# feiyuhuahuo/Yolact_minimal

Measured on NVIDIA B200. Metric: img/s, higher is better.
Workload: dtype f16

## Files before the change

yolact_minimal_b200/csrc/conv_tc.cu:

```cuda
#include "layers.cuh"

#include <cuda.h>
#include <cuda_fp16.h>
#include <stdlib.h>
#include <string.h>
#include <mutex>

namespace yb {

constexpr int TC_BM = 128;
constexpr int TC_BK = 64;
constexpr int TC_THREADS = 320;
constexpr int TC_OUT_BUFS = 2;
constexpr uint32_t TC_WARP_TILE = 32 * 32 * 2;
constexpr uint32_t TC_A_STAGE = TC_BM * TC_BK * 2;
constexpr uint32_t TC_SLAB_ROWS = TC_BM + 2;
constexpr uint32_t TC_A_SLAB = 136 * TC_BK * 2;
constexpr uint32_t TC_S16_ROWS = TC_BM + 3;
constexpr uint32_t TC_S16_SLOT = 5120;

struct TcParams {
  long long M;
  int m_tiles, n_tiles;
  int kb_per_tap;
  int ntaps;
  int tap_shift[kMaxTaps];
  int BN;
  int tmem_cols;
  int stages;
  int Cout, Cout_pad, relu, out_mode;
  int is_f16;
  int tma_epi;
  int nres;
  int b_resident;
  int slab, stages_a;
  int alt_tiles;
  int res_kb;
  int stem16;
  int gemm;
  int gemm_ntile_tap;
  int gemm_shift[16];
  int accumulate;
  int gemm_splits;
  int gemm_kb_split;
  Geom g;
  const float* bias;
  const void* residual;
  void* out;
};

struct TcPlan {
  CUtensorMap tmA, tmB, tmOut, tmRes;
  int BN, stages, tmem_cols, tma_epi, nres, b_resident, res_kb, pair, slab, stages_a, alt_tiles, stem16;
  int sms;
  int gemm;
  size_t smem_bytes;
};

__device__ __forceinline__ uint32_t smem_u32(const void* p) { return (uint32_t)__cvta_generic_to_shared(p); }

__device__ __forceinline__ void mbar_init(uint64_t* bar, uint32_t count) {
  asm volatile("mbarrier.init.shared::cta.b64 [%0], %1;" ::"r"(smem_u32(bar)), "r"(count));
}
__device__ __forceinline__ void mbar_expect_tx(uint64_t* bar, uint32_t bytes) {
  asm volatile("mbarrier.arrive.expect_tx.shared::cta.b64 _, [%0], %1;" ::"r"(smem_u32(bar)), "r"(bytes) : "memory");
}
__device__ __forceinline__ void mbar_arrive(uint64_t* bar) {
  asm volatile("mbarrier.arrive.shared::cta.b64 _, [%0];" ::"r"(smem_u32(bar)) : "memory");
}
__device__ __forceinline__ void mbar_wait(uint64_t* bar, uint32_t parity) {
  asm volatile(
      "{\n\t.reg .pred p;\n\t"
      "WAIT_LOOP:\n\t"
      "mbarrier.try_wait.parity.shared::cta.b64 p, [%0], %1;\n\t"
      "@p bra WAIT_DONE;\n\t"
      "bra WAIT_LOOP;\n\t"
      "WAIT_DONE:\n\t}" ::"r"(smem_u32(bar)), "r"(parity)
// ... 115 lines not shown
__device__ __forceinline__ void tmem_ld16(uint32_t taddr, uint32_t* r) {
  asm volatile(
      "tcgen05.ld.sync.aligned.32x32b.x16.b32 {%0,%1,%2,%3,%4,%5,%6,%7,%8,%9,%10,%11,%12,%13,%14,%15}, [%16];"
      : "=r"(r[0]), "=r"(r[1]), "=r"(r[2]), "=r"(r[3]), "=r"(r[4]), "=r"(r[5]), "=r"(r[6]), "=r"(r[7]), "=r"(r[8]),
        "=r"(r[9]), "=r"(r[10]), "=r"(r[11]), "=r"(r[12]), "=r"(r[13]), "=r"(r[14]), "=r"(r[15])
      : "r"(taddr)
      : "memory");
}
__device__ __forceinline__ void tmem_ld_wait() { asm volatile("tcgen05.wait::ld.sync.aligned;" ::: "memory"); }

template <bool F16> __device__ __forceinline__ uint32_t pack2(float a, float b) {
  if (F16) {
    __half2 v = __floats2half2_rn(fminf(fmaxf(a, -65504.f), 65504.f), fminf(fmaxf(b, -65504.f), 65504.f));
    return *reinterpret_cast<uint32_t*>(&v);
  } else {
    __nv_bfloat162 v = __floats2bfloat162_rn(a, b);
    return *reinterpret_cast<uint32_t*>(&v);
  }
}
template <bool F16, bool RELU> __device__ __forceinline__ uint32_t pack2_sat(float a, float b) {
  uint32_t r;
  if (F16) {
    if (RELU) asm("cvt.rn.relu.satfinite.f16x2.f32 %0, %1, %2;" : "=r"(r) : "f"(b), "f"(a));
    else asm("cvt.rn.satfinite.f16x2.f32 %0, %1, %2;" : "=r"(r) : "f"(b), "f"(a));
  } else {
    if (RELU) asm("cvt.rn.relu.bf16x2.f32 %0, %1, %2;" : "=r"(r) : "f"(b), "f"(a));
    else asm("cvt.rn.bf16x2.f32 %0, %1, %2;" : "=r"(r) : "f"(b), "f"(a));
  }
  return r;
}
template <bool F16> __device__ __forceinline__ float2 unpack2(uint32_t u) {
  if (F16) return __half22float2(*reinterpret_cast<const __half2*>(&u));
  return __bfloat1622float2(*reinterpret_cast<const __nv_bfloat162*>(&u));
}

template <int NCOL, bool F16>
__device__ __forceinline__ void epilogue_chunk(const TcParams& p, const uint32_t* acc, long long m, int col, bool valid, bool halo,
                                               int img, int y, int x) {
  if (!valid) return;
  if (p.out_mode == 2) {
    float* o = (float*)p.out + m * p.Cout_pad + col;
#pragma unroll
    for (int i = 0; i < NCOL; i += 4) {
      const float4 r = make_float4(__uint_as_float(acc[i]), __uint_as_float(acc[i + 1]), __uint_as_float(acc[i + 2]), __uint_as_float(acc[i + 3]));
      if (p.accumulate) atomicAdd(reinterpret_cast<float4*>(o + i), r);
      else *reinterpret_cast<float4*>(o + i) = r;
    }
    return;
  }
  float v[NCOL];
#pragma unroll
  for (int i = 0; i < NCOL; i += 4) {
    const float4 b = __ldg(reinterpret_cast<const float4*>(p.bias + col + i));
    v[i] = __uint_as_float(acc[i]) + b.x; v[i + 1] = __uint_as_float(acc[i + 1]) + b.y;
    v[i + 2] = __uint_as_float(acc[i + 2]) + b.z; v[i + 3] = __uint_as_float(acc[i + 3]) + b.w;
  }
  if (p.out_mode == 0) {
    uint16_t* o = (uint16_t*)p.out + m * p.Cout + col;
    if (halo) {
#pragma unroll
      for (int i = 0; i < NCOL; i += 8) *reinterpret_cast<uint4*>(o + i) = make_uint4(0, 0, 0, 0);
      return;
    }
    if (p.residual) {
      const uint16_t* r = (const uint16_t*)p.residual + m * p.Cout + col;
#pragma unroll
// ... 340 lines not shown
      mbar_expect_tx(&gres_full[buf], TC_WARP_TILE);
      tma_load_2d(gRes + buf * TC_WARP_TILE, &tmRes, pf_nt * p.BN + (2 * pf_j + grp) * 32, pf_mt * TC_BM + quad * 32, &gres_full[buf]);
      ++pf_seq;
      if (++pf_j == my_chunks) { pf_j = 0; ++pf_it; pf_ok = tile_at<PAIR>(p, pf_it, pf_mt, pf_nt); }
    };
    if (elected) {
      for (int q = 0; q < nres && pf_ok; ++q) issue_res_load();
    }
    int m_tile, n_tile;
    for (int it = 0; tile_at<PAIR>(p, it, m_tile, n_tile); ++it) {
      if (p.alt_tiles && (it & 1) != grp) {
        acc ^= 1; if (acc == 0) acc_phase ^= 1;
        continue;
      }
      const long long m = (long long)m_tile * TC_BM + row_in_tile;
      const bool valid = m < p.M;
      int img = 0, y = 0, x = 0;
      bool halo = false;
      if (valid && p.out_mode != 2) {
        const int plane = p.g.plane();
        img = (int)(m / plane);
        const int pos = (int)(m - (long long)img * plane);
        y = pos / p.g.Wp(); x = pos - y * p.g.Wp();
        halo = y == 0 || y == p.g.H + 1 || x == 0 || x == p.g.W + 1;
      }
      mbar_wait(&tmem_full[acc], acc_phase);
      tc_fence_after();
      const uint32_t t_base = tmem_base + ((uint32_t)(quad * 32) << 16) + (uint32_t)(acc * p.BN);
      const int n0 = n_tile * p.BN;
      if (p.tma_epi) {
        const uint32_t sw = (uint32_t)((lane >> 1) & 3);
        const bool zero_row = halo || !valid;
        const int row0 = m_tile * TC_BM + quad * 32;
        uint32_t r[32];
        if (my_chunks > 0) tmem_ld32(t_base + cfirst * 32, r);
        for (int j = 0; j < my_chunks; ++j, ++seq) {
          const int c = cstep * j + cfirst;
          const int col = n0 + c * 32;
          const int obuf = seq & (TC_OUT_BUFS - 1);
          float v[32];
#pragma unroll
          for (int i = 0; i < 32; i += 4) {
            const float4 b = __ldg(reinterpret_cast<const float4*>(p.bias + col + i));
            v[i] = b.x; v[i + 1] = b.y; v[i + 2] = b.z; v[i + 3] = b.w;
          }
          tmem_ld_wait();
#pragma unroll
          for (int i = 0; i < 32; ++i) v[i] += __uint_as_float(r[i]);
          if (j + 1 < my_chunks) tmem_ld32(t_base + (c + cstep) * 32, r);
          if (has_res) {
            const int rbuf = seq & (nres - 1);
            mbar_wait(&gres_full[rbuf], (uint32_t)((seq >> nres_shift) & 1));
            const uint8_t* rrow = gRes + rbuf * TC_WARP_TILE + lane * 64;
#pragma unroll
            for (int jj = 0; jj < 4; ++jj) {
              const uint4 rv = *reinterpret_cast<const uint4*>(rrow + (((uint32_t)jj ^ sw) << 4));
              const uint32_t rw[4] = {rv.x, rv.y, rv.z, rv.w};
#pragma unroll
              for (int q = 0; q < 4; ++q) {
                const float2 f = unpack2<F16>(rw[q]);
                v[jj * 8 + 2 * q] += f.x; v[jj * 8 + 2 * q + 1] += f.y;
              }
            }
          }
          uint32_t pk[16];
          if (p.relu == 1) {
#pragma unroll
            for (int i = 0; i < 16; ++i) pk[i] = pack2_sat<F16, true>(v[2 * i], v[2 * i + 1]);
          } else {
            if (p.relu == 2) {
#pragma unroll
              for (int i = 0; i < 32; ++i) v[i] = apply_act(v[i], 2);
            }
#pragma unroll
            for (int i = 0; i < 16; ++i) pk[i] = pack2_sat<F16, false>(v[2 * i], v[2 * i + 1]);
          }
          if (zero_row) {
#pragma unroll
            for (int i = 0; i < 16; ++i) pk[i] = 0u;
          }
          if (elected) bulk_wait_read<1>();
          __syncwarp();
          uint8_t* orow = gOut + obuf * TC_WARP_TILE + lane * 64;
#pragma unroll
          for (int jj = 0; jj < 4; ++jj)
            *reinterpret_cast<uint4*>(orow + (((uint32_t)jj ^ sw) << 4)) = make_uint4(pk[jj * 4], pk[jj * 4 + 1], pk[jj * 4 + 2], pk[jj * 4 + 3]);
          fence_async_smem();
          __syncwarp();
          if (elected) {
            tma_store_2d(&tmOut, gOut + obuf * TC_WARP_TILE, col, row0);
            bulk_commit();
            if (pf_ok) issue_res_load();
          }
        }
      } else {
        for (int c0 = cfirst * 32; c0 < p.BN; c0 += 32 * cstep) {
          uint32_t r[32];
          if (c0 + 32 <= p.BN) {
            tmem_ld32(t_base + c0, r);
            tmem_ld_wait();
            epilogue_chunk<32, F16>(p, r, m, n0 + c0, valid, halo, img, y, x);
          } else {
            tmem_ld16(t_base + c0, r);
            tmem_ld_wait();
            epilogue_chunk<16, F16>(p, r, m, n0 + c0, valid, halo, img, y, x);
          }
        }
      }
      tc_fence_before();
      __syncwarp();
      if (lane == 0) {
        if (PAIR) mbar_arrive_cluster(map_to_rank(smem_u32(&tmem_empty[acc]), 0)); else mbar_arrive(&tmem_empty[acc]);
      }
      acc ^= 1; if (acc == 0) acc_phase ^= 1;
    }
    if (p.tma_epi && elected) bulk_wait<0>();
  }

  tc_fence_before();
  if (PAIR) cluster_sync_all(); else __syncthreads();
  if (warp == 1) {
    tc_fence_after();
// ... 569 lines not shown
  p.ntaps = 1; p.tap_shift[0] = 0;
  for (int i = 0; i < g.ntaps; ++i) p.gemm_shift[i] = g.shift[i];
  p.BN = pl->BN; p.tmem_cols = pl->tmem_cols; p.stages = pl->stages;
  p.Cout = p.Cout_pad = g.ntaps * g.Nper; p.relu = 0; p.out_mode = 2; p.accumulate = g.accumulate;
  p.is_f16 = g.act_dt == DT_F16; p.alt_tiles = pl->alt_tiles;
  p.g.H = 1 << 20; p.g.W = 1 << 20;
  p.bias = nullptr; p.residual = nullptr; p.out = g.out;
  const int total = p.m_tiles * p.n_tiles * p.gemm_splits;
  const int grid = total < pl->sms ? total : pl->sms;
  cudaLaunchConfig_t cfg = {};
  cfg.gridDim = dim3((unsigned)grid); cfg.blockDim = dim3(TC_THREADS); cfg.dynamicSmemBytes = pl->smem_bytes; cfg.stream = s;
  cfg.attrs = nullptr; cfg.numAttrs = 0;
  const cudaError_t le = p.is_f16 ? cudaLaunchKernelEx(&cfg, k_conv_tc<true, false>, pl->tmA, pl->tmB, pl->tmOut, pl->tmRes, p)
                                  : cudaLaunchKernelEx(&cfg, k_conv_tc<false, false>, pl->tmA, pl->tmB, pl->tmOut, pl->tmRes, p);
  YB_CHECK_CUDA(le);
  YB_CHECK_LAUNCH();
  return YB_OK;
}

int launch_conv_tc(const TcPlan* pl, const ConvArgs& a, cudaStream_t s) {
  TcParams p;
  p.M = (long long)a.B * a.g.plane();
  const int unit_rows = pl->pair ? 2 * TC_BM : TC_BM;
  p.m_tiles = (int)((p.M + unit_rows - 1) / unit_rows);
  p.n_tiles = a.Cout_pad / pl->BN;
  p.kb_per_tap = a.Cin_pad / TC_BK;
  p.ntaps = a.ntaps;
  for (int i = 0; i < kMaxTaps; ++i) p.tap_shift[i] = a.tap_shift[i];
  p.BN = pl->BN; p.tmem_cols = pl->tmem_cols; p.stages = pl->stages;
  p.Cout = a.Cout; p.Cout_pad = a.Cout_pad; p.relu = a.relu; p.out_mode = a.out_mode;
  p.g = a.g; p.bias = a.bias; p.residual = a.residual; p.out = a.out; p.is_f16 = a.act_dt == DT_F16; p.tma_epi = pl->tma_epi; p.nres = pl->nres; p.b_resident = pl->b_resident; p.res_kb = pl->res_kb; p.slab = pl->slab; p.stages_a = pl->stages_a; p.alt_tiles = pl->alt_tiles; p.stem16 = pl->stem16;
  p.gemm = 0; p.gemm_ntile_tap = 1; p.accumulate = 0; p.gemm_splits = 1; p.gemm_kb_split = 0;
  for (int i = 0; i < 16; ++i) p.gemm_shift[i] = 0;
  const int sms = pl->sms;
  const int total = p.m_tiles * p.n_tiles;
  const int max_units = pl->pair ? sms / 2 : sms;
  int units = total < max_units ? total : max_units;
  if (pl->b_resident) {
    units = max_units / p.n_tiles * p.n_tiles;
    if (units > total) units = total;
    if (units < p.n_tiles) units = p.n_tiles;
  }
  const int grid = pl->pair ? 2 * units : units;
  static const bool pdl = getenv("YOLACT_B200_NO_PDL") == nullptr;
  cudaLaunchConfig_t cfg = {};
  cfg.gridDim = dim3((unsigned)grid); cfg.blockDim = dim3(TC_THREADS); cfg.dynamicSmemBytes = pl->smem_bytes; cfg.stream = s;
  cudaLaunchAttribute attr[2];
  int na = 0;
  if (pdl) {
    attr[na].id = cudaLaunchAttributeProgrammaticStreamSerialization;
    attr[na].val.programmaticStreamSerializationAllowed = 1;
    ++na;
  }
  if (pl->pair) {
    attr[na].id = cudaLaunchAttributeClusterDimension;
    attr[na].val.clusterDim.x = 2; attr[na].val.clusterDim.y = 1; attr[na].val.clusterDim.z = 1;
    ++na;
  }
  cfg.attrs = attr; cfg.numAttrs = na;
  cudaError_t le;
  if (pl->pair) le = p.is_f16 ? cudaLaunchKernelEx(&cfg, k_conv_tc<true, true>, pl->tmA, pl->tmB, pl->tmOut, pl->tmRes, p)
                              : cudaLaunchKernelEx(&cfg, k_conv_tc<false, true>, pl->tmA, pl->tmB, pl->tmOut, pl->tmRes, p);
  else le = p.is_f16 ? cudaLaunchKernelEx(&cfg, k_conv_tc<true, false>, pl->tmA, pl->tmB, pl->tmOut, pl->tmRes, p)
                     : cudaLaunchKernelEx(&cfg, k_conv_tc<false, false>, pl->tmA, pl->tmB, pl->tmOut, pl->tmRes, p);
  YB_CHECK_CUDA(le);
  YB_CHECK_LAUNCH();
// ... 96 lines not shown
```

yolact_minimal_b200/csrc/kernels_simt.cu:

```cuda
#include "layers.cuh"
#include <mutex>
#include "vecio.cuh"
#include <math.h>
#include <algorithm>

namespace yb {

__device__ __forceinline__ bool is_halo(long long m, const Geom& g, int& n, int& y, int& x) {
  const int plane = g.plane();
  n = (int)(m / plane);
  const int pos = (int)(m - (long long)n * plane);
  y = pos / g.Wp();
  x = pos - y * g.Wp();
  return y == 0 || y == g.H + 1 || x == 0 || x == g.W + 1;
}

constexpr int SBM = 64, SBN = 64, SBK = 16;

template <typename T>
__global__ void __launch_bounds__(256) k_conv_simt(ConvArgs a, long long M) {
  __shared__ float As[SBK][SBM + 4];
  __shared__ float Bs[SBK][SBN + 4];
  const int tid = threadIdx.x;
  const long long m0 = (long long)blockIdx.x * SBM;
// ... 38 lines not shown
      }
    }
  }
  const T* res = (const T*)a.residual;
#pragma unroll
  for (int i = 0; i < 4; ++i) {
    const long long m = m0 + ty * 4 + i;
    if (m >= M) continue;
    int n, y, x;
    const bool halo = is_halo(m, a.g, n, y, x);
#pragma unroll
    for (int j = 0; j < 4; ++j) {
      const int c = n0 + tx * 4 + j;
      if (c >= a.Cout_pad) continue;
      float v = acc[i][j] + a.bias[c];
      if (a.out_mode == 0) {
        if (c >= a.Cout) continue;
        if (res) v += Act<T>::ld(res + m * a.Cout + c);
        v = apply_act(v, a.relu);
        Act<T>::st((T*)a.out + m * a.Cout + c, halo ? 0.f : v);
      } else if (!halo) {
        v = apply_act(v, a.relu);
        const long long r = ((long long)n * a.g.H + (y - 1)) * a.g.W + (x - 1);
        ((float*)a.out)[r * a.Cout_pad + c] = v;
      }
    }
  }
}

int launch_conv_simt(const ConvArgs& a, cudaStream_t s) {
  const long long M = (long long)a.B * a.g.plane();
  dim3 grid((unsigned)((M + SBM - 1) / SBM), (unsigned)ceil_div(a.Cout_pad, SBN));
  YB_REQUIRE(a.Cin % 4 == 0 && a.Cin_pad % SBK == 0, YB_ERR_UNSUPPORTED, "conv_simt: Cin=%d / Cin_pad=%d", a.Cin, a.Cin_pad);
  YB_DISPATCH_DT(a.act_dt, (k_conv_simt<T><<<grid, 256, 0, s>>>(a, M)));
  YB_CHECK_LAUNCH();
  return YB_OK;
}

constexpr int ST = 16;
constexpr int SP = ST * 2 + 5;

template <typename T>
__global__ void __launch_bounds__(256) k_stem(const float* __restrict__ img, const float* __restrict__ w,
                                              const float* __restrict__ bias, T* __restrict__ out, int S, int H1) {
  extern __shared__ float sm[];
  float* s_w = sm;
  float* s_in = sm + 147 * 64;
  const int tid = threadIdx.x, b = blockIdx.z;
  const int oy0 = blockIdx.y * ST, ox0 = blockIdx.x * ST;
  for (int i = tid; i < 147 * 64; i += 256) s_w[i] = w[i];
  const int iy0 = oy0 * 2 - 3, ix0 = ox0 * 2 - 3;
  for (int i = tid; i < 3 * SP * SP; i += 256) {
    const int c = i / (SP * SP), r = (i / SP) % SP, q = i % SP;
    const int iy = iy0 + r, ix = ix0 + q;
    float v = 0.f;
    if (iy >= 0 && iy < S && ix >= 0 && ix < S) v = img[(((size_t)b * 3 + c) * S + iy) * S + ix];
    s_in[(c * SP + r) * (SP + 1) + q] = v;
  }
  __syncthreads();
  const int py = tid / ST, px = tid % ST;
  const int oy = oy0 + py, ox = ox0 + px;
  float acc[64];
#pragma unroll
  for (int c = 0; c < 64; ++c) acc[c] = 0.f;
  for (int r = 0; r < 7; ++r)
    for (int q = 0; q < 7; ++q)
// ... 458 lines not shown
```

yolact_minimal_b200/csrc/layers.cuh:

```cuda
#pragma once
#include "common.cuh"
#include <cuda_fp16.h>

namespace yb {

enum DType { DT_F32 = 0, DT_BF16 = 1, DT_F16 = 2 };
static inline size_t dtype_size(int dt) { return dt == DT_F32 ? 4 : 2; }

struct Geom {
  int H, W;
  __host__ __device__ int Hp() const { return H + 2; }
  __host__ __device__ int Wp() const { return W + 2; }
  __host__ __device__ int plane() const { return Hp() * Wp(); }
};

constexpr int kMaxTaps = 9;

struct ConvArgs {
  const void* in;
  const void* weight;
  const float* bias;
  const void* residual;
  void* out;
  int act_dt;
  int B;
  Geom g;
  int Cin, Cout, Cout_pad;
  int Cin_pad;
  int ntaps;
  int tap_shift[kMaxTaps];
  int relu;
  int out_mode;
  long long in_rows;
  int in_row_stride;
  long long w_ld;
};

#define YB_DISPATCH_DT(dt, ...)                                   \
  do {                                                            \
    if ((dt) == DT_F32) { using T = float; __VA_ARGS__; }         \
    else if ((dt) == DT_BF16) { using T = __nv_bfloat16; __VA_ARGS__; } \
    else { using T = __half; __VA_ARGS__; }                       \
  } while (0)

int launch_conv_simt(const ConvArgs& a, cudaStream_t s);

struct TcPlan;
int tc_plan_create(const ConvArgs& a_maxbatch, int max_batch, TcPlan** out);
void tc_plan_destroy(TcPlan* p);
int launch_conv_tc(const TcPlan* p, const ConvArgs& a, cudaStream_t s);
bool tc_supported(const ConvArgs& a);

struct GemmArgs {
  const void* a; const void* b; float* out;
  int act_dt, M, Nper, K, lda, ldb, ntaps, accumulate;
  int splits;
  long long Kb;
  int shift[16];
};
int tc_plan_create_gemm(const GemmArgs& g, TcPlan** out);
int launch_gemm_tc(const TcPlan* p, const GemmArgs& g, cudaStream_t s);

struct BneckArgs {
  const void* t2; const void* x; const void* w3; const void* w1;
  const void* xd; int Cd;
  const float* b3; const float* b1;
  void* xo; void* t1;
  int act_dt, B, Cmid, Cexp;
// ... 32 lines not shown
```

yolact_minimal_b200/csrc/net.cu:

```cuda
#include "layers.cuh"

#include <math.h>
#include <stdlib.h>
#include <string.h>
#include <algorithm>
#include <map>
#include <memory>
#include <string>
#include <vector>

using namespace yb;

namespace {

struct Param {
  std::string name;
  int64_t count;
  std::vector<float> data;
  bool set = false;
};

struct ActBuf {
  int C = 0, H = 0;
  int planes = 1;
// ... 1 lines not shown
  size_t bytes = 0;
  int first = 0, last = 0;
  int slot = -1;
  bool dense_f32 = false;
  int pad_rows = 0;
};

enum OpKind { OP_STEM, OP_POOL, OP_SPLIT, OP_CONV, OP_UPADD, OP_UP2X, OP_HEADFIN, OP_PATCH_EMBED, OP_LN, OP_ATTN, OP_MERGE_LN, OP_BNECK };
enum ExtOut { EXT_NONE = 0, EXT_PROTO = 1 };

struct ConvW {
  std::string wname, bname, bnname;
  std::vector<std::string> cat;
  int Cin = 0, Cin_pad = 0, Cout = 0, Cout_pad = 0, k = 1;
  void* d_w = nullptr;
  float* d_b = nullptr;
};

struct Op {
  OpKind kind;
  int in = -1, out = -1, res = -1;
  int conv = -1;
  int stride = 1, relu = 0, out_mode = 0, ext = EXT_NONE;
  int level = 0;
  int aux = -1;
  std::string p0, p1, p2;
  int heads = 0, shift = 0;
  TcPlan* tc = nullptr;
  int conv2 = -1, out2 = -1;
  BnPlan* bn = nullptr;
  int convd = -1, in2 = -1;
  void* d_wcat = nullptr;
  float* d_bcat = nullptr;
};

}

struct yb_net {
  yb_net_config cfg{};
  std::vector<Param> params;
  std::map<std::string, int> pidx;
  std::vector<ActBuf> acts;
  std::vector<ConvW> convs;
  std::vector<Op> ops;
  std::vector<Op> ops_base;
  std::map<std::string, int> taps;
  std::vector<void*> slots;
  std::vector<size_t> slot_bytes;
  bool finalized = false;
  int max_batch = 0, precision = 0, act_dt = DT_F32;
  int H1 = 0, H2 = 0;
  int level_size[5]{}, level_off[5]{};
  int A = 0, P = 0;
  std::vector<float> anchors;
  float* d_anchors = nullptr;
  float* d_stem_w = nullptr;
  float* d_stem_b = nullptr;
  std::map<std::string, float*> d_vec;
  float* d_pe_w = nullptr;
  void* d_stem_w16 = nullptr;
  int stem_wide = 0;
  float* d_stem_b16 = nullptr;
  ConvArgs stem_args{};
  float *d_img = nullptr, *d_cls = nullptr, *d_box = nullptr, *d_coef = nullptr, *d_proto = nullptr;
  void* d_ws = nullptr; size_t ws_bytes = 0;
  int32_t *d_cnt = nullptr, *d_ocls = nullptr, *d_oanc = nullptr; float *d_osc = nullptr, *d_obox = nullptr, *d_ocoef = nullptr;
// ... 245 lines not shown
      const bool ok = ca.k == 1 && cb.k == 1 && a.stride == 1 && b.stride == 1 && a.res >= 0 && b.res < 0 && a.relu == 1 && b.relu == 1 &&
                      a.out_mode == 0 && b.out_mode == 0 && a.ext == EXT_NONE && b.ext == EXT_NONE && b.in == a.out && ca.cat.empty() &&
                      cb.cat.empty() && ca.Cout == cb.Cin && cb.Cout == ca.Cin && ca.Cin == ca.Cin_pad && cb.Cin == cb.Cin_pad &&
                      ca.Cout == ca.Cout_pad && cb.Cout == cb.Cout_pad && bneck_supported(net->act_dt, ca.Cin, ca.Cout);
      if (ok) {
        Op f = a;
        f.kind = OP_BNECK; f.conv2 = b.conv; f.out2 = b.out;
        merged.push_back(f);
        ++i;
        continue;
      }
    }
    merged.push_back(a);
  }
  std::vector<Op> folded;
  for (size_t i = 0; i < merged.size(); ++i) {
    Op f = merged[i];
    if (f.kind == OP_BNECK && !folded.empty() && !getenv("YOLACT_B200_NO_FUSE_DOWN")) {
      const Op& d = folded.back();
      if (d.kind == OP_CONV && d.out == f.res && d.stride == 1 && d.relu == 0 && d.res < 0 && d.out_mode == 0 && d.ext == EXT_NONE) {
        const ConvW& cd = net->convs[d.conv];
        const ConvW& c3 = net->convs[f.conv];
        if (cd.k == 1 && cd.cat.empty() && cd.Cin == cd.Cin_pad && cd.Cout == c3.Cout && (c3.Cin + cd.Cin) / 64 <= 2 && net->acts[d.in].H == net->acts[f.in].H) {
          f.convd = d.conv; f.in2 = d.in; f.res = -1;
          folded.pop_back();
        }
      }
    }
    folded.push_back(f);
  }
  net->ops.swap(folded);
}

void bneck_args(const yb_net* net, const Op& o, int B, BneckArgs* a) {
  const ConvW& c3 = net->convs[o.conv];
  const ConvW& c1 = net->convs[o.conv2];
  memset(a, 0, sizeof(*a));
  a->t2 = net->slots[net->acts[o.in].slot];
  if (o.convd >= 0) { a->xd = net->slots[net->acts[o.in2].slot]; a->Cd = net->convs[o.convd].Cin; }
  else a->x = net->slots[net->acts[o.res].slot];
  a->xo = net->slots[net->acts[o.out].slot]; a->t1 = net->slots[net->acts[o.out2].slot];
  a->w3 = o.convd >= 0 ? o.d_wcat : c3.d_w; a->b3 = o.convd >= 0 ? o.d_bcat : c3.d_b; a->w1 = c1.d_w; a->b1 = c1.d_b;
  a->act_dt = net->act_dt; a->B = B; a->Cmid = c3.Cin; a->Cexp = c3.Cout;
  a->g.H = net->acts[o.in].H; a->g.W = a->g.H;
}

void plan_memory(yb_net* net) {
  auto& acts = net->acts;
  for (auto& a : acts) { a.first = 1 << 30; a.last = -1; }
  for (int i = 0; i < (int)net->ops.size(); ++i) {
    const Op& o = net->ops[i];
    for (int t : {o.in, o.out, o.res, o.aux, o.out2, o.in2}) {
      if (t < 0) continue;
      acts[t].first = acts[t].first < i ? acts[t].first : i;
      acts[t].last = acts[t].last > i ? acts[t].last : i;
    }
  }
  for (auto& kv : net->taps) acts[kv.second].last = 1 << 30;
  const size_t esz = dtype_size(net->act_dt);
  for (auto& a : acts) {
    a.dt = a.dense_f32 ? DT_F32 : net->act_dt;
    const size_t rows = a.dense_f32 ? (size_t)net->max_batch * a.H * a.H : (size_t)net->max_batch * (a.H + 2) * (a.H + 2) * a.planes;
    a.bytes = align_up((rows + a.pad_rows) * a.C * (a.dense_f32 ? 4 : esz), 1024);
  }
  std::vector<int> slot_free_at;
  net->slot_bytes.clear();
// ... 59 lines not shown
      for (int co = 0; co < cout; ++co) bias[row + co] = bb[co];
      row += cout;
    }
  }
  if (net->act_dt == DT_F32) {
    YB_PROPAGATE(upload(w.data(), w.size() * 4, &c.d_w));
  } else if (net->act_dt == DT_BF16) {
    std::vector<__nv_bfloat16> wb(w.size());
    for (size_t i = 0; i < w.size(); ++i) wb[i] = __float2bfloat16_rn(w[i]);
    YB_PROPAGATE(upload(wb.data(), wb.size() * 2, &c.d_w));
  } else {
    std::vector<__half> wb(w.size());
    for (size_t i = 0; i < w.size(); ++i) wb[i] = __float2half_rn(w[i]);
    YB_PROPAGATE(upload(wb.data(), wb.size() * 2, &c.d_w));
  }
  YB_PROPAGATE(upload(bias.data(), bias.size() * 4, (void**)&c.d_b));
  return YB_OK;
}

void* act_ptr(const yb_net* net, int a) { return net->slots[net->acts[a].slot]; }

void conv_args(const yb_net* net, const Op& o, int B, ConvArgs* a, void* ext_out) {
  const ConvW& c = net->convs[o.conv];
  const ActBuf& in = net->acts[o.in];
  memset(a, 0, sizeof(*a));
  a->in = act_ptr(net, o.in);
  a->weight = c.d_w; a->bias = c.d_b;
  a->residual = o.res >= 0 ? act_ptr(net, o.res) : nullptr;
  a->out = o.ext != EXT_NONE ? ext_out : act_ptr(net, o.out);
  a->act_dt = net->act_dt; a->B = B;
  a->g.H = in.H; a->g.W = in.H;
  a->Cin = c.Cin; a->Cin_pad = c.Cin_pad; a->Cout = c.Cout; a->Cout_pad = c.Cout_pad;
  a->relu = o.relu; a->out_mode = o.out_mode;
  const int Wp = in.H + 2;
  const long long plane_rows = (long long)net->max_batch * Wp * Wp;
  a->in_rows = plane_rows * in.planes;
  if (o.stride == 1) {
    a->ntaps = c.k * c.k;
    for (int r = 0; r < c.k; ++r)
      for (int s = 0; s < c.k; ++s) a->tap_shift[r * c.k + s] = c.k == 1 ? 0 : (r - 1) * Wp + (s - 1);
    a->in_rows = (long long)B * Wp * Wp;
  } else if (c.k == 1) {
    a->ntaps = 1; a->tap_shift[0] = 0;
  } else {
    a->ntaps = 9;
    for (int r = 0; r < 3; ++r)
      for (int s = 0; s < 3; ++s) {
        const int pr = r == 1 ? 0 : 1, ps = s == 1 ? 0 : 1, dy = r == 0 ? -1 : 0, dx = s == 0 ? -1 : 0;
        a->tap_shift[r * 3 + s] = (int)((pr * 2 + ps) * plane_rows) + dy * Wp + dx;
      }
  }
}

}

extern "C" int yb_net_create(const yb_net_config* cfg, yb_net** out) {
  YB_REQUIRE(cfg && out, YB_ERR_INVALID, "yb_net_create: NULL argument");
  YB_REQUIRE(cfg->depth == 50 || cfg->depth == 101 || cfg->depth == 0, YB_ERR_UNSUPPORTED, "yb_net_create: depth=%d (50, 101, or 0 = Swin-T)", cfg->depth);
  YB_REQUIRE(cfg->img_size >= 64 && cfg->img_size <= 4096, YB_ERR_INVALID, "yb_net_create: img_size=%d", cfg->img_size);
  YB_REQUIRE(cfg->num_classes >= 2 && cfg->num_ratios >= 1 && cfg->num_ratios <= 3, YB_ERR_INVALID, "yb_net_create: num_classes=%d num_ratios=%d", cfg->num_classes, cfg->num_ratios);
  YB_REQUIRE(cfg->coef_dim > 0 && cfg->coef_dim % 4 == 0 && cfg->coef_dim <= 64, YB_ERR_UNSUPPORTED, "yb_net_create: coef_dim=%d", cfg->coef_dim);
  yb_net* net = new yb_net();
  net->cfg = *cfg;
  build_program(net);
  net->ops_base = net->ops;
  *out = net;
// ... 30 lines not shown
extern "C" int yb_net_set_param(yb_net* net, const char* name, const float* data, int64_t count) {
  YB_REQUIRE(net && name && data, YB_ERR_INVALID, "yb_net_set_param: NULL argument");
  auto it = net->pidx.find(name);
  YB_REQUIRE(it != net->pidx.end(), YB_ERR_INVALID, "yb_net_set_param: unexpected parameter '%s'", name);
  Param& p = net->params[it->second];
  YB_REQUIRE(p.count == count, YB_ERR_INVALID, "yb_net_set_param: '%s' has %lld elements, expected %lld", name, (long long)count, (long long)p.count);
  p.data.assign(data, data + count);
  p.set = true;
  net->finalized = false;
  return YB_OK;
}

extern "C" int yb_net_finalize(yb_net* net, int max_batch, int precision) {
  YB_REQUIRE(net, YB_ERR_INVALID, "yb_net_finalize: NULL net");
  YB_REQUIRE(max_batch >= 1 && max_batch <= 4096, YB_ERR_INVALID, "yb_net_finalize: max_batch=%d", max_batch);
  YB_REQUIRE(precision == YB_PREC_FP32 || precision == YB_PREC_BF16 || precision == YB_PREC_FP16, YB_ERR_INVALID, "yb_net_finalize: precision=%d", precision);
  for (const auto& p : net->params)
    YB_REQUIRE(p.set, YB_ERR_STATE, "yb_net_finalize: parameter '%s' was never set (strict load)", p.name.c_str());
  int cc_major = 0;
  YB_PROPAGATE(yb_device_info(nullptr, &cc_major, nullptr));
  YB_REQUIRE(cc_major == 10, YB_ERR_UNSUPPORTED, "yb_net_finalize: this library is built for sm_100a only (device cc major %d)", cc_major);
  net->drop_graphs();
  for (void* p : net->slots) cudaFree(p);
  net->slots.clear();
  for (auto& c : net->convs) { cudaFree(c.d_w); cudaFree(c.d_b); c.d_w = nullptr; c.d_b = nullptr; }
  for (auto& o : net->ops) { tc_plan_destroy(o.tc); bneck_plan_destroy(o.bn); cudaFree(o.d_wcat); cudaFree(o.d_bcat); }
  net->ops = net->ops_base;
  cudaFree(net->d_anchors); cudaFree(net->d_stem_w); cudaFree(net->d_stem_b); cudaFree(net->d_stem_w16); cudaFree(net->d_stem_b16);
  net->d_anchors = net->d_stem_w = net->d_stem_b = net->d_stem_b16 = nullptr; net->d_stem_w16 = nullptr;

  net->max_batch = max_batch; net->precision = precision;
  net->act_dt = precision == YB_PREC_BF16 ? DT_BF16 : (precision == YB_PREC_FP16 ? DT_F16 : DT_F32);
  fuse_bottlenecks(net);
  plan_memory(net);
  net->slots.resize(net->slot_bytes.size(), nullptr);
  for (size_t s = 0; s < net->slot_bytes.size(); ++s) {
    YB_CHECK_CUDA(cudaMalloc(&net->slots[s], net->slot_bytes[s]));
    YB_CHECK_CUDA(cudaMemset(net->slots[s], 0, net->slot_bytes[s]));
  }
  for (auto& c : net->convs) YB_PROPAGATE(pack_conv(net, c));
  for (auto& kv : net->d_vec) cudaFree(kv.second);
  net->d_vec.clear();
  cudaFree(net->d_pe_w); net->d_pe_w = nullptr;
  if (net->cfg.depth == 0) {
    for (const Op& o : net->ops)
      for (const std::string* nm : {&o.p0, &o.p1})
        if (!nm->empty() && !net->d_vec.count(*nm)) { float* d = nullptr; const auto& v = net->P_(*nm); YB_PROPAGATE(upload(v.data(), v.size() * 4, (void**)&d)); net->d_vec[*nm] = d; }
    for (const char* nm : {"backbone.patch_embed.proj.bias", "backbone.patch_embed.norm.weight", "backbone.patch_embed.norm.bias"}) {
      float* d = nullptr; const auto& v = net->P_(nm); YB_PROPAGATE(upload(v.data(), v.size() * 4, (void**)&d)); net->d_vec[nm] = d;
    }
    const auto& src = net->P_("backbone.patch_embed.proj.weight");
    std::vector<float> w(48 * 96);
    for (int co = 0; co < 96; ++co) for (int k = 0; k < 48; ++k) w[k * 96 + co] = src[co * 48 + k];
    YB_PROPAGATE(upload(w.data(), w.size() * 4, (void**)&net->d_pe_w));
  } else {
    std::vector<float> s, t, w(147 * 64);
    bn_fold(net, "backbone.bn1", 64, s, t);
    const auto& src = net->P_("backbone.conv1.weight");
    for (int co = 0; co < 64; ++co)
      for (int ci = 0; ci < 3; ++ci)
        for (int r = 0; r < 7; ++r)
          for (int q = 0; q < 7; ++q) w[((r * 7 + q) * 3 + ci) * 64 + co] = src[((co * 3 + ci) * 7 + r) * 7 + q] * s[co];
    YB_PROPAGATE(upload(w.data(), w.size() * 4, (void**)&net->d_stem_w));
    YB_PROPAGATE(upload(t.data(), t.size() * 4, (void**)&net->d_stem_b));
  }
  YB_PROPAGATE(upload(net->anchors.data(), net->anchors.size() * 4, (void**)&net->d_anchors));
// ... 168 lines not shown

extern "C" int yb_net_set_profiling(yb_net* net, int enable) {
  YB_REQUIRE(net, YB_ERR_INVALID, "yb_net_set_profiling: NULL net");
  net->profiling = enable != 0;
  return YB_OK;
}

extern "C" int yb_net_profile(yb_net* net, yb_prof_entry* out, int max_entries, int* num_entries) {
  YB_REQUIRE(net && out && num_entries, YB_ERR_INVALID, "yb_net_profile: NULL argument");
  static const char* kNames[] = {"conv_tc", "conv_simt", "stem", "maxpool", "phase_split", "upsample_add", "upsample2x", "head_finalize",
                                 "patch_embed", "layernorm", "window_attention", "patch_merge_ln", "bneck_tc"};
  const int NK = 13;
  YB_REQUIRE(max_entries >= NK, YB_ERR_INVALID, "yb_net_profile: need room for %d entries", NK);
  for (int i = 0; i < NK; ++i) { memset(&out[i], 0, sizeof(out[i])); strncpy(out[i].name, kNames[i], sizeof(out[i].name) - 1); }
  const size_t esz = dtype_size(net->act_dt);
  FILE* dump = nullptr;
  if (const char* path = getenv("YOLACT_B200_PROFILE_DUMP")) dump = fopen(path, "w");
  if (dump) fprintf(dump, "forward,op,kind,tc,cin,cout,k,stride,h_out,batch,ms,gflop\n");
  for (size_t f = 0; f < net->prof_sets.size(); ++f) {
    auto& evs = net->prof_sets[f];
    const double B = net->prof_batch[f];
    YB_CHECK_CUDA(cudaEventSynchronize(evs.back()));
    for (size_t i = 0; i < net->ops.size(); ++i) {
      const Op& o = net->ops[i];
      float ms = 0.f;
      YB_CHECK_CUDA(cudaEventElapsedTime(&ms, evs[i], evs[i + 1]));
      int k = 0; double flops = 0, bytes = 0;
      switch (o.kind) {
        case OP_CONV: {
          const ConvW& c = net->convs[o.conv];
          const double Ho = net->acts[o.in].H, px = B * Ho * Ho;
          k = o.tc ? 0 : 1;
          flops = 2.0 * px * c.Cout * c.Cin * c.k * c.k;
          bytes = px * c.Cin * esz * (o.stride == 2 && c.k == 3 ? 4 : 1) + (double)c.Cout * c.Cin * c.k * c.k * esz +
                  px * c.Cout * (o.out_mode == 1 ? 4 : esz) + (o.res >= 0 ? px * c.Cout * esz : 0);
          break;
        }
        case OP_BNECK: {
          const ConvW& c3 = net->convs[o.conv];
          const double Ho = net->acts[o.in].H, px = B * Ho * Ho;
          k = 12;
          flops = 4.0 * px * c3.Cout * c3.Cin;
          bytes = px * esz * (2.0 * c3.Cin + 2.0 * c3.Cout) + 2.0 * c3.Cout * c3.Cin * esz;
          if (o.convd >= 0) {
            const double Cd = net->convs[o.convd].Cin;
            flops += 2.0 * px * c3.Cout * Cd;
            bytes += px * esz * (Cd - c3.Cout) + c3.Cout * Cd * esz;
          }
          break;
        }
        case OP_STEM: k = 2; flops = 2.0 * B * net->H1 * net->H1 * 64 * 147; bytes = B * 3.0 * net->cfg.img_size * net->cfg.img_size * 4 + B * net->H1 * net->H1 * 64.0 * esz; break;
        case OP_POOL: k = 3; bytes = B * 64.0 * esz * ((double)net->H1 * net->H1 + (double)net->H2 * net->H2); break;
        case OP_SPLIT: { k = 4; const ActBuf& a = net->acts[o.out]; bytes = 2.0 * B * a.H * a.H * a.planes * a.C * esz; break; }
        case OP_UPADD: { k = 5; const ActBuf& a = net->acts[o.out]; bytes = 2.25 * B * a.H * a.H * a.C * esz; break; }
        case OP_UP2X: { k = 6; const ActBuf& a = net->acts[o.out]; bytes = 1.25 * B * a.H * a.H * a.C * esz; break; }
        case OP_HEADFIN: { k = 7; const ActBuf& a = net->acts[o.in]; bytes = 2.0 * B * a.H * a.H * a.C * 4; break; }
        case OP_PATCH_EMBED: { k = 8; const ActBuf& a = net->acts[o.out]; flops = 2.0 * B * a.H * a.H * 96 * 48; bytes = B * 3.0 * net->cfg.img_size * net->cfg.img_size * 4 + B * a.H * a.H * 96.0 * esz; break; }
        case OP_LN: { k = 9; const ActBuf& a = net->acts[o.out]; bytes = 2.0 * B * a.H * a.H * a.C * esz; break; }
        case OP_ATTN: { k = 10; const ActBuf& a = net->acts[o.out]; const double nw = ((a.H + 6) / 7) * ((a.H + 6) / 7);
                        flops = B * nw * o.heads * 4.0 * 49 * 49 * 32; bytes = 4.0 * B * a.H * a.H * a.C * esz; break; }
        case OP_MERGE_LN: { k = 11; const ActBuf& a = net->acts[o.out]; bytes = 2.0 * B * a.H * a.H * a.C * esz; break; }
      }
      if (dump) {
        const ConvW* c = (o.kind == OP_CONV || o.kind == OP_BNECK) ? &net->convs[o.conv] : nullptr;
        fprintf(dump, "%zu,%zu,%d,%d,%d,%d,%d,%d,%d,%d,%.5f,%.4f\n", f, i, (int)o.kind, o.tc ? 1 : 0, c ? c->Cin : 0, c ? c->Cout_pad : 0,
                c ? c->k : 0, o.stride, c ? net->acts[o.in].H : 0, (int)B, ms, flops * 1e-9);
      }
      out[k].launches += (o.kind == OP_STEM ? 2 : 1);
// ... 275 lines not shown
```

Before: 4906.

## Fold parity-plane split into producing conv epilogue

Removes separate OP_SPLIT ops by having the preceding stride-1 tensor-core conv write its output directly into four parity-split padded planes. The epilogue switches from TMA stores to per-lane scattered 16B global stores, computed from each row's plane coordinates, and writes zeros into the halo rows of the split layout. This saves a full read and write of the activation plus a kernel launch, at the cost of uncoalesced-ish stores that lose TMA's bulk-store efficiency.

Result: no change. 4915, median of 6 (+0.2%).

```diff
diff --git a/yolact_minimal_b200/csrc/conv_tc.cu b/yolact_minimal_b200/csrc/conv_tc.cu
--- a/yolact_minimal_b200/csrc/conv_tc.cu
+++ b/yolact_minimal_b200/csrc/conv_tc.cu
@@ -43,6 +43,8 @@
   int accumulate;
   int gemm_splits;
   int gemm_kb_split;
+  int split_H;
+  long long split_rows;
   Geom g;
   const float* bias;
   const void* residual;
@@ -224,6 +226,12 @@
 template <bool F16> __device__ __forceinline__ float2 unpack2(uint32_t u) {
   if (F16) return __half22float2(*reinterpret_cast<const __half2*>(&u));
   return __bfloat1622float2(*reinterpret_cast<const __nv_bfloat162*>(&u));
+}
+
+__device__ __forceinline__ long long plane_row(const TcParams& p, int img, int iy, int ix) {
+  const int Hpo = p.split_H + 2;
+  const int pl = (iy & 1) * 2 + (ix & 1);
+  return (long long)pl * p.split_rows + ((long long)img * Hpo + (iy >> 1) + 1) * Hpo + (ix >> 1) + 1;
 }
 
 template <int NCOL, bool F16>
@@ -630,6 +638,12 @@
         const uint32_t sw = (uint32_t)((lane >> 1) & 3);
         const bool zero_row = halo || !valid;
         const int row0 = m_tile * TC_BM + quad * 32;
+        long long srow[4] = {-1, -1, -1, -1};
+        if (p.split_H) {
+          const long long own = valid ? plane_row(p, img, y - 1, x - 1) : -1;
+#pragma unroll
+          for (int k = 0; k < 4; ++k) srow[k] = __shfl_sync(0xffffffffu, own, 8 * k + (lane >> 2));
+        }
         uint32_t r[32];
         if (my_chunks > 0) tmem_ld32(t_base + cfirst * 32, r);
         for (int j = 0; j < my_chunks; ++j, ++seq) {
@@ -685,7 +699,30 @@
             *reinterpret_cast<uint4*>(orow + (((uint32_t)jj ^ sw) << 4)) = make_uint4(pk[jj * 4], pk[jj * 4 + 1], pk[jj * 4 + 2], pk[jj * 4 + 3]);
           fence_async_smem();
           __syncwarp();
-          if (elected) {
+          if (p.split_H) {
+            const uint8_t* sbuf = gOut + obuf * TC_WARP_TILE;
+            const int piece = lane & 3;
+#pragma unroll
+            for (int k = 0; k < 4; ++k) {
+              const int rr = 8 * k + (lane >> 2);
+              if (srow[k] >= 0)
+                *reinterpret_cast<uint4*>((uint16_t*)p.out + srow[k] * p.Cout + col + piece * 8) =
+                    *reinterpret_cast<const uint4*>(sbuf + rr * 64 + (((uint32_t)piece ^ ((rr >> 1) & 3)) << 4));
+            }
+            const int iy = y - 1, ix = x - 1;
+            if (valid && (iy == -1 || iy == p.g.H || ix == -1 || ix == p.g.W)) {
+              const int last = 2 * p.split_H + 1;
+              const int ylo = iy == -1 ? -2 : iy, yhi = iy == p.g.H ? last : iy;
+              const int xlo = ix == -1 ? -2 : ix, xhi = ix == p.g.W ? last : ix;
+              for (int yy = ylo; yy <= yhi; ++yy)
+                for (int xx = xlo; xx <= xhi; ++xx) {
+                  if (yy == iy && xx == ix) continue;
+                  uint4* o = reinterpret_cast<uint4*>((uint16_t*)p.out + plane_row(p, img, yy, xx) * p.Cout + col);
+#pragma unroll
+                  for (int jj = 0; jj < 4; ++jj) o[jj] = make_uint4(0u, 0u, 0u, 0u);
+                }
+            }
+          } else if (elected) {
             tma_store_2d(&tmOut, gOut + obuf * TC_WARP_TILE, col, row0);
             bulk_commit();
             if (pf_ok) issue_res_load();
@@ -1321,6 +1358,9 @@
   p.g = a.g; p.bias = a.bias; p.residual = a.residual; p.out = a.out; p.is_f16 = a.act_dt == DT_F16; p.tma_epi = pl->tma_epi; p.nres = pl->nres; p.b_resident = pl->b_resident; p.res_kb = pl->res_kb; p.slab = pl->slab; p.stages_a = pl->stages_a; p.alt_tiles = pl->alt_tiles; p.stem16 = pl->stem16;
   p.gemm = 0; p.gemm_ntile_tap = 1; p.accumulate = 0; p.gemm_splits = 1; p.gemm_kb_split = 0;
   for (int i = 0; i < 16; ++i) p.gemm_shift[i] = 0;
+  p.split_H = a.split_H; p.split_rows = a.split_rows;
+  YB_REQUIRE(!a.split_H || (pl->tma_epi && !a.residual), YB_ERR_UNSUPPORTED,
+             "launch_conv_tc: the parity-plane epilogue needs the TMA epilogue form and no residual (Cout_pad=%d)", a.Cout_pad);
   const int sms = pl->sms;
   const int total = p.m_tiles * p.n_tiles;
   const int max_units = pl->pair ? sms / 2 : sms;
diff --git a/yolact_minimal_b200/csrc/kernels_simt.cu b/yolact_minimal_b200/csrc/kernels_simt.cu
--- a/yolact_minimal_b200/csrc/kernels_simt.cu
+++ b/yolact_minimal_b200/csrc/kernels_simt.cu
@@ -94,6 +94,7 @@
   const long long M = (long long)a.B * a.g.plane();
   dim3 grid((unsigned)((M + SBM - 1) / SBM), (unsigned)ceil_div(a.Cout_pad, SBN));
   YB_REQUIRE(a.Cin % 4 == 0 && a.Cin_pad % SBK == 0, YB_ERR_UNSUPPORTED, "conv_simt: Cin=%d / Cin_pad=%d", a.Cin, a.Cin_pad);
+  YB_REQUIRE(!a.split_H, YB_ERR_UNSUPPORTED, "conv_simt: no parity-plane epilogue (tensor-core path only)");
   YB_DISPATCH_DT(a.act_dt, (k_conv_simt<T><<<grid, 256, 0, s>>>(a, M)));
   YB_CHECK_LAUNCH();
   return YB_OK;
diff --git a/yolact_minimal_b200/csrc/layers.cuh b/yolact_minimal_b200/csrc/layers.cuh
--- a/yolact_minimal_b200/csrc/layers.cuh
+++ b/yolact_minimal_b200/csrc/layers.cuh
@@ -34,6 +34,8 @@
   long long in_rows;
   int in_row_stride;
   long long w_ld;
+  int split_H;
+  long long split_rows;
 };
 
 #define YB_DISPATCH_DT(dt, ...)                                   \
diff --git a/yolact_minimal_b200/csrc/net.cu b/yolact_minimal_b200/csrc/net.cu
--- a/yolact_minimal_b200/csrc/net.cu
+++ b/yolact_minimal_b200/csrc/net.cu
@@ -57,6 +57,7 @@
   int convd = -1, in2 = -1;
   void* d_wcat = nullptr;
   float* d_bcat = nullptr;
+  int split = 0;
 };
 
 }
@@ -368,6 +369,34 @@
   net->ops.swap(folded);
 }
 
+void fold_glue(yb_net* net) {
+  if (net->act_dt == DT_F32 || getenv("YOLACT_B200_NO_TC") || getenv("YOLACT_B200_NO_FOLD")) return;
+  auto& ops = net->ops;
+  auto readers = [&](int act) {
+    int n = 0;
+    for (const Op& o : ops)
+      for (int t : {o.in, o.res, o.aux, o.in2}) n += t == act;
+    return n;
+  };
+  auto foldable = [&](const Op& o) {
+    if (o.kind != OP_CONV || o.stride != 1 || o.res >= 0 || o.out_mode != 0 || o.ext != EXT_NONE) return false;
+    const ConvW& c = net->convs[o.conv];
+    ConvArgs a; memset(&a, 0, sizeof(a));
+    a.act_dt = net->act_dt; a.Cin = c.Cin; a.Cin_pad = c.Cin_pad; a.Cout = c.Cout; a.Cout_pad = c.Cout_pad;
+    return tc_supported(a) && c.Cout % 32 == 0;
+  };
+  for (size_t i = 1; i < ops.size(); ++i) {
+    const Op s = ops[i];
+    Op& prod = ops[i - 1];
+    if (s.kind != OP_SPLIT || prod.out != s.in || net->acts[s.out].planes != 4 || !foldable(prod) || readers(s.in) != 1) continue;
+    bool tap = false;
+    for (auto& kv : net->taps) tap |= kv.second == s.in;
+    if (tap) continue;
+    prod.out = s.out; prod.split = 1;
+    ops.erase(ops.begin() + i); --i;
+  }
+}
+
 void bneck_args(const yb_net* net, const Op& o, int B, BneckArgs* a) {
   const ConvW& c3 = net->convs[o.conv];
   const ConvW& c1 = net->convs[o.conv2];
@@ -493,6 +522,10 @@
   a->g.H = in.H; a->g.W = in.H;
   a->Cin = c.Cin; a->Cin_pad = c.Cin_pad; a->Cout = c.Cout; a->Cout_pad = c.Cout_pad;
   a->relu = o.relu; a->out_mode = o.out_mode;
+  if (o.split) {
+    const int Ho = net->acts[o.out].H;
+    a->split_H = Ho; a->split_rows = (long long)net->max_batch * (Ho + 2) * (Ho + 2);
+  }
   const int Wp = in.H + 2;
   const long long plane_rows = (long long)net->max_batch * Wp * Wp;
   a->in_rows = plane_rows * in.planes;
@@ -589,6 +622,7 @@
   net->max_batch = max_batch; net->precision = precision;
   net->act_dt = precision == YB_PREC_BF16 ? DT_BF16 : (precision == YB_PREC_FP16 ? DT_F16 : DT_F32);
   fuse_bottlenecks(net);
+  fold_glue(net);
   plan_memory(net);
   net->slots.resize(net->slot_bytes.size(), nullptr);
   for (size_t s = 0; s < net->slot_bytes.size(); ++s) {
@@ -823,8 +857,9 @@
           const double Ho = net->acts[o.in].H, px = B * Ho * Ho;
           k = o.tc ? 0 : 1;
           flops = 2.0 * px * c.Cout * c.Cin * c.k * c.k;
+          const double Hs = net->acts[o.out].H, px_out = o.split ? 4.0 * B * Hs * Hs : px;
           bytes = px * c.Cin * esz * (o.stride == 2 && c.k == 3 ? 4 : 1) + (double)c.Cout * c.Cin * c.k * c.k * esz +
-                  px * c.Cout * (o.out_mode == 1 ? 4 : esz) + (o.res >= 0 ? px * c.Cout * esz : 0);
+                  px_out * c.Cout * (o.out_mode == 1 ? 4 : esz) + (o.res >= 0 ? px * c.Cout * esz : 0);
           break;
         }
         case OP_BNECK: {
```
